# indianajohn/akaze-rust

Measured on AMD Instinct MI355X. Metric: Mpix/s through extract_features (4 oct x 4 sub), higher is better.
Workload: dtype f32

## Files before the change

### akaze-rust_amd/csrc/akz_kernels.hip

```cpp
#include <hip/hip_runtime.h>

#include <algorithm>
#include <cstdlib>

#include "akz_internal.hpp"
#include "akz_pm_g2.hpp"
#include "akz_libm.hpp"
#include "akz_prep_passes.hpp"

namespace akz {
namespace {

constexpr int BX = 64, BY = 4;

__device__ __forceinline__ int clampi(int v, int lo, int hi) { return v < lo ? lo : (v > hi ? hi : v); }

__device__ __forceinline__ float px(const float* p, long i) { return p[i]; }
__device__ __forceinline__ float px(const uint8_t* p, long i) { return ((float)p[i] * 1.0f) / 255.0f; }

template <typename T>
__global__ void k_filter_h(const T* __restrict__ in, float* __restrict__ out, int w, int h, Taps t) {
    const int x = blockIdx.x * BX + threadIdx.x, y = blockIdx.y * BY + threadIdx.y;
    if (x >= w || y >= h) return;
    const size_t base = (size_t)blockIdx.z * (size_t)w * (size_t)h;
// ... 319 lines not shown
            if (ly < n || ly >= n + TH || gy >= h || gx >= w) continue;
            const float* v = r == 0 ? la : lb;
            const float* st = r == 0 ? sta : stb;
            float* po = L_out + base + (size_t)gy * w;
            float* ps = Lstep ? Lstep + base + (size_t)gy * w : nullptr;
            if (vec_ok && gx + 3 < w) {
                plane_store4(po + gx, v[0], v[1], v[2], v[3]);
                if (ps) plane_store4(ps + gx, st[0], st[1], st[2], st[3]);
            } else {
#pragma unroll
                for (int e = 0; e < 4; ++e)
                    if (gx + e < w) {
                        plane_store(po + gx + e, v[e]);
                        if (ps) plane_store(ps + gx + e, st[e]);
                    }
            }
        }
    }
    if constexpr (EPI) {
        constexpr int IW = TW + 4, IH = TH + 4;
        static_assert(IH * IW + (TH + 4) * (TW + 2) + (TH + 2) * (TW + 2) <= 2 * PLANE, "the preparation's windows fit the two planes");
        float* const wI = sAB;
        float* const wA = wI + IH * IW;
        float* const wB = wA + (TH + 4) * (TW + 2);
        __syncthreads();
        if (active) {
#pragma unroll
            for (int r = 0; r < 2; ++r) {
                const int gy = r == 0 ? gya : gyb;
                const int wy = gy - (y0 - 2);
                if (wy < 0 || wy >= IH || gy < 0 || gy >= h) continue;
                const float* v = r == 0 ? la : lb;
#pragma unroll
                for (int e = 0; e < 4; ++e) {
                    const int wx = gx + e - (x0 - 2);
                    if (wx >= 0 && wx < IW && gx + e >= 0 && gx + e < w) wI[wy * IW + wx] = v[e];
                }
            }
        }
        __syncthreads();
        const double kc = octave_contrast(ep.d_k[blockIdx.z], ep.k_pow);
        prep_passes<TW, TH, NT>(wI, wA, wB, x0, y0, w, h, base, ep.lsmooth, ep.lflow, ep.taps, 1.0 / (kc * kc));
    }
}

__device__ __forceinline__ double grad_mod(const float* I, int w, int h, int x, int y, Scharr1 sk) {
    float lx, ly;
    scharr1_pair(I, w, h, x, y, sk, lx, ly);
    const double dx = (double)lx, dy = (double)ly;
    return sqrt(dx * dx + dy * dy);
}
constexpr int CT = 256;
__global__ void __launch_bounds__(CT)
k_contrast_max(const float* __restrict__ blurred, int w, int h, Scharr1 sk,
               unsigned long long* __restrict__ d_hmax_bits) {
    __shared__ unsigned long long s_part[CT / 64];
    const float* I = blurred + (size_t)blockIdx.z * (size_t)w * (size_t)h;
    double m = 0.0;
    for (int y = 1 + (int)blockIdx.x; y < h - 1; y += (int)gridDim.x)
        for (int x = 1 + (int)threadIdx.x; x < w - 1; x += CT) {
            const double g = grad_mod(I, w, h, x, y, sk);
            if (g > m) m = g;
        }
    unsigned long long bits = (unsigned long long)__double_as_longlong(m);
    for (int o = 32; o > 0; o >>= 1) {
        const unsigned long long other = __shfl_xor(bits, o, 64);
        bits = other > bits ? other : bits;
    }
    if ((threadIdx.x & 63) == 0) s_part[threadIdx.x >> 6] = bits;
    __syncthreads();
    if (threadIdx.x == 0) {
        for (int i = 1; i < CT / 64; ++i) bits = s_part[i] > bits ? s_part[i] : bits;
        if (bits != 0ull) atomicMax(d_hmax_bits + blockIdx.z, bits);
    }
}
__global__ void __launch_bounds__(CT)
k_contrast_hist(const float* __restrict__ blurred, int w, int h, Scharr1 sk,
                const unsigned long long* __restrict__ d_hmax_bits, unsigned nbins, unsigned copies,
                unsigned* __restrict__ d_hist) {
    extern __shared__ unsigned s_hist[];
    const unsigned tid = threadIdx.x;
    for (unsigned b = tid; b < nbins * copies; b += CT) s_hist[b] = 0u;
    __syncthreads();
    const float* I = blurred + (size_t)blockIdx.z * (size_t)w * (size_t)h;
    const double hmax = __longlong_as_double((long long)d_hmax_bits[blockIdx.z]);
    unsigned* mine = s_hist + (tid & (copies - 1u)) * nbins;
    for (int y = 1 + (int)blockIdx.x; y < h - 1; y += (int)gridDim.x)
        for (int x = 1 + (int)tid; x < w - 1; x += CT) {
            const double g = grad_mod(I, w, h, x, y, sk);
            if (g != 0.0) {
                const double f = floor((double)nbins * (g / hmax));
                const unsigned b = f >= (double)nbins ? nbins - 1u : (f > 0.0 ? (unsigned)f : 0u);
                atomicAdd(&mine[b], 1u);
            }
        }
    __syncthreads();
    for (unsigned b = tid; b < nbins; b += CT) {
        unsigned v = 0;
        for (unsigned c = 0; c < copies; ++c) v += s_hist[c * nbins + b];
        if (v) atomicAdd(&d_hist[(size_t)blockIdx.z * nbins + b], v);
    }
}
__device__ __forceinline__ unsigned long long sat_usize(double v) {
    if (!(v > 0.0)) return 0ull;
    if (v >= 18446744073709551615.0) return ~0ull;
    return (unsigned long long)v;
}
__global__ void __launch_bounds__(256)
k_contrast_final(const unsigned long long* __restrict__ d_hmax_bits, const unsigned* __restrict__ d_hist,
                 unsigned nbins, double percentile, unsigned n, double* __restrict__ d_k) {
    extern __shared__ unsigned s_bins[];
    const unsigned img = blockIdx.x;
    if (img >= n) return;
    const unsigned* hist = d_hist + (size_t)img * nbins;
    for (unsigned b = threadIdx.x; b < nbins; b += blockDim.x) s_bins[b] = hist[b];
    __syncthreads();
    if (threadIdx.x != 0) return;
    const double hmax = __longlong_as_double((long long)d_hmax_bits[img]);
    unsigned long long num_points = 0;
    for (unsigned b = 0; b < nbins; ++b) num_points += s_bins[b];
    const unsigned long long threshold = sat_usize((double)num_points * percentile);
    unsigned long long k = 0, num_elements = 0;
    while (num_elements < threshold && k < nbins) {
        num_elements += s_bins[k];
        k += 1;
    }
    d_k[img] = num_elements >= threshold ? hmax * (double)k / (double)nbins : 0.03;
}

template <int NTH>
__global__ void __launch_bounds__(NTH)
k_contrast_hist_final(const float* __restrict__ gxp, const float* __restrict__ gyp, int w, int h, unsigned long long* __restrict__ d_smax_bits,
                      unsigned nbins, unsigned copies, unsigned* __restrict__ d_hist, unsigned* __restrict__ d_done, double percentile,
                      double* __restrict__ d_k) {
    extern __shared__ unsigned s_hist[];
    __shared__ unsigned s_last;
    const unsigned tid = threadIdx.x, img = blockIdx.z;
    for (unsigned b = tid; b < nbins * copies; b += NTH) s_hist[b] = 0u;
    __syncthreads();
    const size_t px = (size_t)w * (size_t)h;
    const float* GX = gxp + (size_t)img * px;
    const float* GY = gyp + (size_t)img * px;
    const double hmax = sqrt(__longlong_as_double((long long)d_smax_bits[img]));
    unsigned* mine = s_hist + (tid & (copies - 1u)) * nbins;
    const bool vec = (px & 3u) == 0;
    const size_t nquads = (px + 3) / 4;
    for (size_t q = (size_t)blockIdx.x * NTH + tid; q < nquads; q += (size_t)gridDim.x * NTH) {
        const size_t i0 = q * 4;
        float ax[4], ay[4];
        if (vec) {
            const float4 a = *reinterpret_cast<const float4*>(GX + i0), b = *reinterpret_cast<const float4*>(GY + i0);
            ax[0] = a.x; ax[1] = a.y; ax[2] = a.z; ax[3] = a.w;
            ay[0] = b.x; ay[1] = b.y; ay[2] = b.z; ay[3] = b.w;
        } else {
#pragma unroll
            for (int e = 0; e < 4; ++e) {
                ax[e] = i0 + e < px ? GX[i0 + e] : 0.0f;
                ay[e] = i0 + e < px ? GY[i0 + e] : 0.0f;
            }
        }
        int y = (int)(i0 / (size_t)w), x = (int)(i0 - (size_t)y * w);
#pragma unroll
        for (int e = 0; e < 4; ++e) {
            if (x >= 1 && x < w - 1 && y >= 1 && y < h - 1) {
                const double dx = (double)ax[e], dy = (double)ay[e];
                const double g = sqrt(dx * dx + dy * dy);
                if (g != 0.0) {
                    const double f = floor((double)nbins * (g / hmax));
                    const unsigned b = f >= (double)nbins ? nbins - 1u : (f > 0.0 ? (unsigned)f : 0u);
                    atomicAdd(&mine[b], 1u);
                }
            }
            if (++x == w) {
                x = 0;
                ++y;
            }
        }
    }
    __syncthreads();
    unsigned* hist = d_hist + (size_t)img * nbins;
    for (unsigned b = tid; b < nbins; b += NTH) {
        unsigned v = 0;
        for (unsigned c = 0; c < copies; ++c) v += s_hist[c * nbins + b];
        if (v) {
            const unsigned before = atomicAdd(&hist[b], v);
            asm volatile("" ::"v"(before));
        }
    }
    __builtin_amdgcn_fence(__ATOMIC_RELEASE, "workgroup");
    __builtin_amdgcn_s_waitcnt(0);
    __syncthreads();
    if (tid == 0) s_last = atomicAdd(&d_done[img], 1u) == gridDim.x - 1u ? 1u : 0u;
    __syncthreads();
    if (!s_last) return;
    for (unsigned b = tid; b < nbins; b += NTH) {
        s_hist[b] = __hip_atomic_load(&hist[b], __ATOMIC_RELAXED, __HIP_MEMORY_SCOPE_AGENT);
        hist[b] = 0u;
    }
    __syncthreads();
    if (tid != 0) return;
    unsigned long long num_points = 0;
    for (unsigned b = 0; b < nbins; ++b) num_points += s_hist[b];
    const unsigned long long threshold = sat_usize((double)num_points * percentile);
    unsigned long long k = 0, num_elements = 0;
    while (num_elements < threshold && k < nbins) {
        num_elements += s_hist[k];
        k += 1;
    }
    d_k[img] = num_elements >= threshold ? hmax * (double)k / (double)nbins : 0.03;
    d_smax_bits[img] = 0ull;
    d_done[img] = 0u;
}
__global__ void __launch_bounds__(256)
k_flow_pair(const float* __restrict__ gxp, const float* __restrict__ gyp, float* __restrict__ lflow, size_t px, const double* __restrict__ d_k,
            unsigned k_pow) {
    const unsigned img = blockIdx.z;
    const double kc = octave_contrast(d_k[img], k_pow);
    const double inverse_k = 1.0 / (kc * kc);
    const float* GX = gxp + (size_t)img * px;
    const float* GY = gyp + (size_t)img * px;
    float* out = lflow + (size_t)img * px;
    const size_t i0 = ((size_t)blockIdx.x * 256 + threadIdx.x) * 4;
    if (i0 >= px) return;
    if ((px & 3u) == 0) {
        const float4 a = *reinterpret_cast<const float4*>(GX + i0), b = *reinterpret_cast<const float4*>(GY + i0);
        float4 o;
        o.x = pm_g2_px(a.x, b.x, inverse_k);
        o.y = pm_g2_px(a.y, b.y, inverse_k);
        o.z = pm_g2_px(a.z, b.z, inverse_k);
        o.w = pm_g2_px(a.w, b.w, inverse_k);
        *reinterpret_cast<float4*>(out + i0) = o;
    } else {
        for (size_t i = i0; i < i0 + 4 && i < px; ++i) out[i] = pm_g2_px(GX[i], GY[i], inverse_k);
    }
}

__global__ void k_ldet(const float* __restrict__ lxx, const float* __restrict__ lyy, const float* __restrict__ lxy,
                       float* __restrict__ out, size_t count, float q) {
    const size_t i = (size_t)blockIdx.x * blockDim.x + threadIdx.x;
    if (i >= count) return;
    out[i] = ((lxx[i] * lyy[i]) - (lxy[i] * lxy[i])) * q;
}

__global__ void k_accumulate(float* a, const float* b, size_t count) {
    const size_t i = (size_t)blockIdx.x * blockDim.x + threadIdx.x;
    if (i >= count) return;
    a[i] = a[i] + b[i];
}

__device__ __forceinline__ void nms_emit(float v, float xp, float xm, float yp, float ym, int x, int y, int w, int h,
                                         unsigned level, unsigned img, float thr, float border_m,
                                         Candidate* __restrict__ cand, unsigned cap, unsigned* __restrict__ count) {
    if (!(v > thr)) return;
    if (!(v > xp && v > xm && v > ym && v > yp)) return;
    const float fx = (float)x, fy = (float)y;
    const bool is_out = (roundf(fx - border_m) - 1.0f) < 0.0f || (roundf(fx + border_m) + 1.0f) >= (float)w ||
                        (roundf(fy - border_m) - 1.0f) < 0.0f || (roundf(fy + border_m) + 1.0f) >= (float)h;
    if (is_out) return;
    const unsigned slot = atomicAdd(count, 1u);
    if (slot < cap) {
        Candidate c;
        c.level = level;
        c.idx = (unsigned)(y * w + x);
        c.v = v; c.xp = xp; c.xm = xm; c.yp = yp; c.ym = ym;
        c.img = img;
        cand[slot] = c;
    }
}
__global__ void k_nms(const float* __restrict__ ldet, int w, int h, size_t img_stride, unsigned level, float thr,
                      float border_m, Candidate* __restrict__ cand, unsigned cap, unsigned* __restrict__ count) {
    const int x0 = (blockIdx.x * BX + threadIdx.x) * 4, y = blockIdx.y * BY + threadIdx.y;
    if (x0 >= w || y < 1 || y >= h - 1) return;
    const float* D = ldet + (size_t)blockIdx.z * img_stride;
    const float* row = D + (size_t)y * w;
    float c[6], up[4], dn[4];
    if ((w & 3) == 0 && x0 + 3 < w) {
        const float4 vc = *reinterpret_cast<const float4*>(row + x0);
        const float4 vu = *reinterpret_cast<const float4*>(row - w + x0);
        const float4 vd = *reinterpret_cast<const float4*>(row + w + x0);
        c[1] = vc.x; c[2] = vc.y; c[3] = vc.z; c[4] = vc.w;
        up[0] = vu.x; up[1] = vu.y; up[2] = vu.z; up[3] = vu.w;
        dn[0] = vd.x; dn[1] = vd.y; dn[2] = vd.z; dn[3] = vd.w;
    } else {
#pragma unroll
        for (int e = 0; e < 4; ++e) {
            const bool in = x0 + e < w;
            c[e + 1] = in ? row[x0 + e] : 0.0f;
            up[e] = in ? row[x0 + e - w] : 0.0f;
            dn[e] = in ? row[x0 + e + w] : 0.0f;
        }
    }
    c[0] = x0 > 0 ? row[x0 - 1] : 0.0f;
    c[5] = (x0 + 4 < w) ? row[x0 + 4] : 0.0f;
    const long last = (long)w * h - w - 1;
#pragma unroll
    for (int e = 0; e < 4; ++e) {
        const int x = x0 + e;
        if (x < 1 || x >= w) continue;
        if ((long)y * w + x >= last) continue;
        nms_emit(c[e + 1], c[e + 2], c[e], dn[e], up[e], x, y, w, h, level, blockIdx.z, thr, border_m, cand, cap, count);
    }
}

__constant__ float c_gauss25[7][7] = {
    {0.02546481f, 0.02350698f, 0.01849125f, 0.01239505f, 0.00708017f, 0.00344629f, 0.00142946f},
    {0.02350698f, 0.02169968f, 0.01706957f, 0.01144208f, 0.00653582f, 0.00318132f, 0.00131956f},
    {0.01849125f, 0.01706957f, 0.01342740f, 0.00900066f, 0.00514126f, 0.00250252f, 0.00103800f},
    {0.01239505f, 0.01144208f, 0.00900066f, 0.00603332f, 0.00344629f, 0.00167749f, 0.00069579f},
    {0.00708017f, 0.00653582f, 0.00514126f, 0.00344629f, 0.00196855f, 0.00095820f, 0.00039744f},
    {0.00344629f, 0.00318132f, 0.00250252f, 0.00167749f, 0.00095820f, 0.00046640f, 0.00019346f},
    {0.00142946f, 0.00131956f, 0.00103800f, 0.00069579f, 0.00039744f, 0.00019346f, 0.00008024f}};

struct OriTable {
    signed char a[112], b[112];
};
constexpr OriTable make_ori_table() {
    OriTable t{};
    int idx = 0;
    for (int i = -6; i <= 6; ++i)
        for (int j = -6; j <= 6; ++j)
            if (i * i + j * j < 36) {
                t.a[idx] = (signed char)i;
                t.b[idx] = (signed char)j;
                ++idx;
            }
    for (; idx < 112; ++idx) { t.a[idx] = 0; t.b[idx] = 0; }
    return t;
}
__constant__ OriTable c_ori = make_ori_table();
struct OriOrder {
    unsigned char k[112];
};
constexpr OriOrder make_ori_order() {
    OriOrder o{};
    const OriTable t = make_ori_table();
    int n = 0;
    for (int b = -6; b <= 6; ++b)
        for (int a = -6; a <= 6; ++a)
            for (int k = 0; k < 109; ++k)
                if (t.a[k] == a && t.b[k] == b) o.k[n++] = (unsigned char)k;
    for (; n < 112; ++n) o.k[n] = 0;
    return o;
}
__constant__ OriOrder c_ori_rows = make_ori_order();

__device__ __forceinline__ unsigned xcd_contiguous_group(unsigned b, unsigned nb) {
    return (b & 7u) * (nb >> 3) + (b >> 3);
}

constexpr int ORI_KPB = 32, ORI_NS = 109, ORI_NT = 256;
__global__ void __launch_bounds__(ORI_NT)
k_orientation(LevelTable tab, const KpParam* __restrict__ kps, unsigned nkp, const unsigned* __restrict__ d_nkp,
              unsigned long long window_mask, unsigned n_windows, OrientOut* __restrict__ out, unsigned out_stride) {
    __shared__ float s_rx[ORI_KPB * ORI_NS];
    __shared__ float s_ry[ORI_KPB * ORI_NS + 16];
    if (d_nkp) nkp = min(nkp, *d_nkp);
    const unsigned base = xcd_contiguous_group(blockIdx.x, gridDim.x) * ORI_KPB;
    if (base >= nkp) return;
    constexpr int ORI_IT = (ORI_KPB * ORI_NS + ORI_NT - 1) / ORI_NT, ORI_UB = 7;
    static_assert(ORI_IT % ORI_UB == 0, "whole batches");
    for (int it0 = 0; it0 < ORI_IT; it0 += ORI_UB) {
        float vx[ORI_UB], vy[ORI_UB], gw[ORI_UB];
        unsigned slot[ORI_UB];
#pragma unroll
        for (int u = 0; u < ORI_UB; ++u) {
            const unsigned idx = threadIdx.x + (unsigned)(it0 + u) * ORI_NT;
            const unsigned j = idx / ORI_NS, k = c_ori_rows.k[idx - j * ORI_NS];
            vx[u] = 0.0f; vy[u] = 0.0f; gw[u] = 0.0f;
            slot[u] = j * ORI_NS + k;
            if (idx < ORI_KPB * ORI_NS && base + j < nkp) {
                const KpParam kp = kps[base + j];
                const LevelPtrs lv = tab.lv[kp.level];
                const float* lx = lv.lx + (size_t)kp.img * lv.stride;
                const float* ly = lv.ly + (size_t)kp.img * lv.stride;
                const int a = c_ori.a[k], b = c_ori.b[k];
                const float fy = roundf(kp.yf + (float)b * kp.scale);
                const float fx = roundf(kp.xf + (float)a * kp.scale);
                const int iy = clampi(fy > 0.0f ? (int)fy : 0, 0, (int)lv.h - 1);
                const int ix = clampi(fx > 0.0f ? (int)fx : 0, 0, (int)lv.w - 1);
                gw[u] = c_gauss25[a < 0 ? -a : a][b < 0 ? -b : b];
                const size_t p = (size_t)iy * lv.w + ix;
                vx[u] = lx[p];
                vy[u] = ly[p];
            }
        }
#pragma unroll
        for (int u = 0; u < ORI_UB; ++u) {
            const unsigned idx = threadIdx.x + (unsigned)(it0 + u) * ORI_NT;
            const unsigned j = idx / ORI_NS;
            if (idx < ORI_KPB * ORI_NS) {
                const bool have = base + j < nkp;
                s_rx[slot[u]] = have ? gw[u] * vx[u] : 0.0f;
                s_ry[slot[u]] = have ? gw[u] * vy[u] : 0.0f;
            }
        }
    }
    __syncthreads();
    if (threadIdx.x >= 64) return;
    const unsigned lane = threadIdx.x, j = lane >> 1;
    const bool is_y = (lane & 1u) != 0;
    const float* py = s_ry + j * ORI_NS;
    const float* pa = is_y ? py : s_rx + j * ORI_NS;
    float t[ORI_NS];
#pragma unroll
    for (int k = 0; k < ORI_NS; ++k) t[k] = py[k] > 0.0f ? pa[k] : -0.0f;
    float sum = 0.0f, maxv = 0.0f, bx = 0.0f, by = 0.0f;
    unsigned found = 0;
    for (unsigned wdw = 0; wdw < n_windows; ++wdw) {
        if ((window_mask >> wdw) & 1ull) {
#pragma unroll
            for (int k = 0; k < ORI_NS; ++k) sum = sum + t[k];
        }
        const float other = __shfl_xor(sum, 1, 64);
        const float sx = is_y ? other : sum, sy = is_y ? sum : other;
        const float val = sx * sx + sy * sy;
        if (val > maxv) {
            maxv = val;
            bx = sx;
            by = sy;
            found = 1;
        }
    }
    if (!is_y && base + j < nkp) {
        OrientOut o;
        o.sum_x = bx; o.sum_y = by; o.found = found; o.angle_bits = 0;
        out[(size_t)(base + j) * out_stride] = o;
    }
}

struct PairTable {
    unsigned char a[162], b[162];
};
constexpr PairTable make_pairs() {
    PairTable t{};
    int p = 0;
    const int counts[3] = {4, 9, 16}, base[3] = {0, 4, 13};
    for (int g = 0; g < 3; ++g)
        for (int i = 0; i < counts[g]; ++i)
            for (int j = i + 1; j < counts[g]; ++j) {
                t.a[p] = (unsigned char)(base[g] + i);
                t.b[p] = (unsigned char)(base[g] + j);
                ++p;
            }
    return t;
}
__constant__ PairTable c_pairs = make_pairs();
struct BitTable3 {
    unsigned short e[512];
};
constexpr BitTable3 make_bits3() {
    BitTable3 t{};
    const PairTable p = make_pairs();
    const int npairs[3] = {6, 36, 120}, pbase[3] = {0, 6, 42};
    int b = 0;
    for (int g = 0; g < 3; ++g)
        for (int pos = 0; pos < 3; ++pos)
            for (int q = 0; q < npairs[g]; ++q)
                t.e[b++] = (unsigned short)((pos << 10) | (p.a[pbase[g] + q] << 5) | p.b[pbase[g] + q]);
    for (; b < 512; ++b) t.e[b] = 0;
    return t;
}
__constant__ BitTable3 c_bits3 = make_bits3();

constexpr int MLDB_KPB = 4;
constexpr int MLDB_LAT = 21, MLDB_NS = MLDB_LAT * MLDB_LAT;
struct DeviceAngles {
    OrientOut* sums;
    unsigned stride;
    unsigned fma;
    unsigned* flag;
};
struct MldbHostMirror {
    uint4* recs;
    const uint4* hdr;
    uint4* hdr_host;
    unsigned hdr_vec;
    uint8_t* desc;
};
__device__ __forceinline__ float2 device_angle(const DeviceAngles& da, unsigned kpi, bool write, const MldbHostMirror& hm) {
    OrientOut* o = da.sums + (size_t)kpi * da.stride;
    const float ang = o->found ? libm::atan2f_glibc(o->sum_y, o->sum_x) : 0.0f;
    bool bad = false;
    float co, si;
    if (da.fma) {
        co = libm::cosf_glibc<true>(ang, &bad);
        si = libm::sinf_glibc<true>(ang, &bad);
    } else {
        co = libm::cosf_glibc<false>(ang, &bad);
        si = libm::sinf_glibc<false>(ang, &bad);
    }
    if (write) {
        o->angle_bits = __float_as_uint(ang);
        if (bad && da.flag) atomicOr(da.flag, 1u);
        if (hm.recs) {
            const uint4* rec = reinterpret_cast<const uint4*>(da.sums) + (size_t)kpi * 2u - 1u;
            uint4 r0 = rec[0], r1 = rec[1];
            r1.w = __float_as_uint(ang);
            hm.recs[(size_t)kpi * 2u] = r0;
            hm.recs[(size_t)kpi * 2u + 1u] = r1;
        }
    }
    return float2{co, si};
}
__global__ void __launch_bounds__(64 * MLDB_KPB)
k_mldb(LevelTable tab, const KpParam* __restrict__ kps, const float2* __restrict__ cosi, unsigned nkp, const unsigned* __restrict__ d_nkp,
       DeviceAngles da, unsigned channels, uint8_t* __restrict__ desc64, unsigned first, MldbHostMirror hm) {
    __shared__ float s_win[MLDB_KPB][3][MLDB_NS + 7];
    __shared__ float s_val[MLDB_KPB][3][32];
    if (hm.recs && blockIdx.x == 0)
        for (unsigned i = threadIdx.x; i < hm.hdr_vec; i += 64 * MLDB_KPB) hm.hdr_host[i] = hm.hdr[i];
    if (d_nkp) nkp = min(nkp, *d_nkp);
    const unsigned lane = threadIdx.x & 63u, wv = threadIdx.x >> 6;
    const unsigned group0 = first + xcd_contiguous_group(blockIdx.x, gridDim.x) * MLDB_KPB;
    const unsigned kpi = group0 + wv;
    if (group0 >= nkp) return;
    const bool live = kpi < nkp;
    KpParam kp = kps[live ? kpi : 0];
    const float2 cs = da.sums ? device_angle(da, live ? kpi : 0, live && lane == 0, hm) : cosi[live ? kpi : 0];
    const LevelPtrs lv = tab.lv[__builtin_amdgcn_readfirstlane(kp.level)];
    const size_t ioff = (size_t)kp.img * lv.stride;
    const float* Lt = lv.lt + ioff;
    const float* Lx = lv.lx + ioff;
    const float* Ly = lv.ly + ioff;
    const float co = cs.x, si = cs.y, scale = kp.scale;
    unsigned short bits3[8];
#pragma unroll
    for (int r = 0; r < 8; ++r) bits3[r] = c_bits3.e[r * 64 + (int)lane];
    if (live) {
        constexpr int NIT = (MLDB_NS + 63) / 64;
        const bool k_fast = fabsf(co) >= fabsf(si);
        unsigned pidx[NIT];
        int widx[NIT];
#pragma unroll
        for (int it = 0; it < NIT; ++it) {
            const int sidx = min((int)lane + 64 * it, MLDB_NS - 1);
            const int qa = sidx / MLDB_LAT, qb = sidx - qa * MLDB_LAT;
            const int kk = k_fast ? qb : qa, ll = k_fast ? qa : qb;
            const int k = kk - 10, l = ll - 10;
            const float lf = (float)l + 0.5f, kf = (float)k + 0.5f;
            const float sample_y = kp.yf + (lf * co * scale + kf * si * scale);
            const float sample_x = kp.xf + (-lf * si * scale + kf * co * scale);
            const int y1 = clampi((int)roundf(sample_y), 0, (int)lv.h - 1);
            const int x1 = clampi((int)roundf(sample_x), 0, (int)lv.w - 1);
            pidx[it] = (unsigned)y1 * (unsigned)lv.w + (unsigned)x1;
            widx[it] = kk * MLDB_LAT + ll;
        }
        float vt[NIT], vx[NIT], vy[NIT];
#pragma unroll
        for (int it = 0; it < NIT; ++it) {
            vt[it] = Lt[pidx[it]];
            vx[it] = channels > 1 ? Lx[pidx[it]] : 0.0f;
            vy[it] = channels > 1 ? Ly[pidx[it]] : 0.0f;
        }
#pragma unroll
        for (int it = 0; it < NIT; ++it) {
            const int sidx = (int)lane + 64 * it;
            if (sidx >= MLDB_NS) continue;
            float v1 = 0.0f, v2 = 0.0f;
            if (channels > 1) {
                const float rx = vx[it], ry = vy[it];
                if (channels == 2) {
                    v1 = sqrtf(rx * rx + ry * ry);
                } else {
                    v2 = rx * co + ry * si;
                    v1 = -rx * si + ry * co;
                }
            }
            s_win[wv][0][widx[it]] = vt[it];
            s_win[wv][1][widx[it]] = v1;
            s_win[wv][2][widx[it]] = v2;
        }
    }
    __syncthreads();
    const unsigned cl = lane & 31u, ckp = 2u * wv + (lane >> 5);
    if (wv < MLDB_KPB / 2 && cl < 29 && group0 + ckp < nkp) {
        const int g = cl < 4 ? 0 : (cl < 13 ? 1 : 2);
        const int step = g == 0 ? 10 : (g == 1 ? 7 : 5), ng = g + 2;
        const int ci = (int)cl - (g == 0 ? 0 : (g == 1 ? 4 : 13));
        const int kk0 = (ci / ng) * step, ll0 = (ci % ng) * step;
        const int per_cell = step * step;
        const float* b0 = &s_win[ckp][0][0];
        const float* b1 = &s_win[ckp][1][0];
        const float* b2 = &s_win[ckp][2][0];
        float di = 0.0f, dx = 0.0f, dy = 0.0f;
#pragma unroll
        for (int dk = 0; dk < 10; ++dk) {
            const int o = (kk0 + min(dk, step - 1)) * MLDB_LAT + ll0;
            float r0[10], r1[10], r2[10];
#pragma unroll
            for (int dl = 0; dl < 10; ++dl) {
                r0[dl] = b0[o + dl];
                r1[dl] = b1[o + dl];
                r2[dl] = b2[o + dl];
            }
#pragma unroll
            for (int dl = 0; dl < 10; ++dl)
                if (dk < step && dl < step) {
                    di = di + r0[dl];
                    dx = dx + r1[dl];
                    dy = dy + r2[dl];
                }
        }
        const float ns = (float)per_cell;
        s_val[ckp][0][cl] = di / ns;
        s_val[ckp][1][cl] = dx / ns;
        s_val[ckp][2][cl] = dy / ns;
    }
    __syncthreads();
    const unsigned seg0 = 6u * channels, seg1 = seg0 + 36u * channels, total = seg1 + 120u * channels;
    unsigned long long words[8];
#pragma unroll
    for (int r = 0; r < 8; ++r) {
        const unsigned b = (unsigned)r * 64u + lane;
        bool bit = false;
        if (channels == 3) {
            const unsigned e = bits3[r];
            bit = s_val[wv][e >> 10][(e >> 5) & 31u] > s_val[wv][e >> 10][e & 31u];
        } else if (b < total) {
            unsigned rel, npairs, pbase;
            if (b < seg0) { rel = b; npairs = 6; pbase = 0; }
            else if (b < seg1) { rel = b - seg0; npairs = 36; pbase = 6; }
            else { rel = b - seg1; npairs = 120; pbase = 42; }
            const unsigned pos = rel / npairs, p = rel % npairs;
            bit = s_val[wv][pos][c_pairs.a[pbase + p]] > s_val[wv][pos][c_pairs.b[pbase + p]];
        }
        words[r] = __ballot(bit);
    }
    if (live && lane < 8) {
        unsigned long long wvw = words[0];
#pragma unroll
        for (int r = 1; r < 8; ++r)
            if (lane == (unsigned)r) wvw = words[r];
        reinterpret_cast<unsigned long long*>(desc64 + (size_t)kpi * 64)[lane] = wvw;
        if (hm.desc) reinterpret_cast<unsigned long long*>(hm.desc + (size_t)kpi * 64)[lane] = wvw;
    }
}

constexpr int MT = 256;

__device__ __forceinline__ unsigned hamming64(const uint4 (&q)[4], const uint4* __restrict__ row, unsigned tail_mask) {
    unsigned d = 0;
#pragma unroll
    for (int k = 0; k < 4; ++k) {
        const uint4 t = row[k];
        d += __popc(q[k].x ^ t.x);
        d += __popc(q[k].y ^ t.y);
        d += __popc(q[k].z ^ t.z);
        d += __popc((q[k].w ^ t.w) & (k == 3 ? tail_mask : 0xffffffffu));
    }
    return d;
}
__device__ __forceinline__ void top2_feed(unsigned d, unsigned j, unsigned& min_d, unsigned& second, unsigned& min_j) {
    if (d < min_d) {
        second = min_d;
        min_d = d;
        min_j = j;
    } else if (d < second) {
        second = d;
    }
}
__global__ void __launch_bounds__(MT) k_match(const uint4* __restrict__ d0, unsigned n0, const uint4* __restrict__ d1,
                                             unsigned n1, unsigned chunk_rows, unsigned threshold, unsigned tail_mask,
                                             MatchRec* __restrict__ out) {
    __shared__ uint4 s_tile[MT * 4];
    const unsigned i = blockIdx.x * MT + threadIdx.x;
    uint4 q[4];
    const bool live = i < n0;
#pragma unroll
    for (int k = 0; k < 4; ++k) q[k] = live ? d0[(size_t)i * 4 + k] : make_uint4(0, 0, 0, 0);
    unsigned min_d = threshold, second = threshold, min_j = 0;
    const unsigned begin = blockIdx.y * chunk_rows, end = min(n1, begin + chunk_rows);
    for (unsigned base = begin; base < end; base += MT) {
        const unsigned rows = min((unsigned)MT, end - base);
        __syncthreads();
        for (unsigned e = threadIdx.x; e < rows * 4; e += MT) s_tile[e] = d1[(size_t)base * 4 + e];
        __syncthreads();
        unsigned r = 0;
        for (; r + 4 <= rows; r += 4) {
            const unsigned da = hamming64(q, s_tile + (r + 0) * 4, tail_mask), db = hamming64(q, s_tile + (r + 1) * 4, tail_mask);
            const unsigned dc = hamming64(q, s_tile + (r + 2) * 4, tail_mask), dd = hamming64(q, s_tile + (r + 3) * 4, tail_mask);
            top2_feed(da, base + r + 0, min_d, second, min_j);
            top2_feed(db, base + r + 1, min_d, second, min_j);
            top2_feed(dc, base + r + 2, min_d, second, min_j);
            top2_feed(dd, base + r + 3, min_d, second, min_j);
        }
        for (; r < rows; ++r) top2_feed(hamming64(q, s_tile + r * 4, tail_mask), base + r, min_d, second, min_j);
    }
    if (live) {
        MatchRec m;
        m.min_d = min_d; m.second_d = second; m.min_j = min_j; m._pad = 0;
        out[(size_t)blockIdx.y * n0 + i] = m;
    }
}
__global__ void k_match_merge(const MatchRec* __restrict__ part, unsigned n0, unsigned chunks, unsigned threshold,
                              MatchRec* __restrict__ out) {
    const unsigned i = blockIdx.x * blockDim.x + threadIdx.x;
    if (i >= n0) return;
    unsigned min_d = threshold, second = threshold, min_j = 0;
    for (unsigned c = 0; c < chunks; ++c) {
        const MatchRec m = part[(size_t)c * n0 + i];
        top2_feed(m.min_d, m.min_j, min_d, second, min_j);
        if (m.second_d < second) second = m.second_d;
    }
    MatchRec o;
    o.min_d = min_d; o.second_d = second; o.min_j = min_j; o._pad = 0;
    out[i] = o;
}

__global__ void __launch_bounds__(1024) k_match_compact(const MatchRec* __restrict__ rec, unsigned n0, unsigned chunks,
                                                        unsigned threshold, double ratio2,
                                                        akz_match* __restrict__ out,
                                                        unsigned long long* __restrict__ n_out) {
    constexpr int IT = 16;
    __shared__ unsigned s_cnt[IT][16];
    __shared__ unsigned s_base;
    rec += (size_t)blockIdx.x * chunks * n0;
    out += (size_t)blockIdx.x * n0;
    n_out += blockIdx.x;
    const unsigned lane = threadIdx.x & 63u, wave = threadIdx.x >> 6;
    if (threadIdx.x == 0) s_base = 0;
    __syncthreads();
    for (unsigned start = 0; start < n0; start += IT * 1024u) {
        unsigned md[IT], mj[IT], keepmask = 0u;
#pragma unroll
        for (int it = 0; it < IT; ++it) {
            const unsigned i = start + (unsigned)it * 1024u + threadIdx.x;
            bool keep = false;
            md[it] = mj[it] = 0u;
            if (i < n0) {
                unsigned min_d = threshold, second = threshold, min_j = 0;
                for (unsigned c = 0; c < chunks; ++c) {
                    const MatchRec p = rec[(size_t)c * n0 + i];
                    top2_feed(p.min_d, p.min_j, min_d, second, min_j);
                    if (p.second_d < second) second = p.second_d;
                }
                md[it] = min_d; mj[it] = min_j;
                keep = ((double)min_d < (double)second * ratio2) && (min_d < threshold);
            }
            const unsigned long long bal = __ballot(keep);
            if (lane == 0) s_cnt[it][wave] = (unsigned)__popcll(bal);
            keepmask |= keep ? 1u << it : 0u;
        }
        __syncthreads();
        unsigned off = s_base;
#pragma unroll
        for (int it = 0; it < IT; ++it) {
            unsigned row = 0, below = 0;
#pragma unroll
            for (unsigned w = 0; w < 16; ++w) {
                const unsigned c = s_cnt[it][w];
                row += c;
                below += w < wave ? c : 0u;
            }
            const bool keep = (keepmask >> it) & 1u;
            const unsigned long long bal = __ballot(keep);
            if (keep) {
                akz_match o;
                o.index_0 = start + (unsigned)it * 1024u + threadIdx.x; o.index_1 = mj[it]; o.distance = (double)md[it];
                out[off + below + (unsigned)__popcll(bal & ((1ull << lane) - 1ull))] = o;
            }
            off += row;
        }
        __syncthreads();
        if (threadIdx.x == 0) s_base = off;
        __syncthreads();
    }
    if (threadIdx.x == 0) *n_out = s_base;
}

__global__ void __launch_bounds__(256) k_match_merge_compact(const MatchRec* __restrict__ part, unsigned n0, unsigned chunks,
                                                             unsigned threshold, double ratio2, akz_match* __restrict__ out,
                                                             unsigned long long* __restrict__ n_out,
                                                             unsigned long long* __restrict__ state, unsigned epoch) {
    __shared__ unsigned s_cnt[4];
    __shared__ unsigned s_prefix;
    const unsigned b = blockIdx.x, tid = threadIdx.x, lane = tid & 63u, wave = tid >> 6;
    const unsigned i = b * 256u + tid;
    unsigned min_d = threshold, second = threshold, min_j = 0;
    bool keep = false;
    if (i < n0) {
        for (unsigned c = 0; c < chunks; ++c) {
            const MatchRec m = part[(size_t)c * n0 + i];
            top2_feed(m.min_d, m.min_j, min_d, second, min_j);
            if (m.second_d < second) second = m.second_d;
        }
        keep = ((double)min_d < (double)second * ratio2) && (min_d < threshold);
    }
    const unsigned long long bal = __ballot(keep);
    if (lane == 0) s_cnt[wave] = (unsigned)__popcll(bal);
    __syncthreads();
    const unsigned total = s_cnt[0] + s_cnt[1] + s_cnt[2] + s_cnt[3];
    unsigned below = 0;
    for (unsigned w = 0; w < wave; ++w) below += s_cnt[w];
    if (tid == 0)
        __hip_atomic_store(state + b, ((unsigned long long)epoch << 32) | total, __ATOMIC_RELAXED, __HIP_MEMORY_SCOPE_AGENT);
    if (wave == 0) {
        unsigned sum = 0;
        for (unsigned j0 = 0; j0 < b; j0 += 64u) {
            const unsigned j = j0 + lane;
            unsigned v = 0;
            if (j < b) {
                unsigned long long w;
                do {
                    w = __hip_atomic_load(state + j, __ATOMIC_RELAXED, __HIP_MEMORY_SCOPE_AGENT);
                } while ((unsigned)(w >> 32) != epoch);
                v = (unsigned)w;
            }
            for (int o = 32; o > 0; o >>= 1) v += __shfl_xor(v, o, 64);
            sum += v;
        }
        if (lane == 0) s_prefix = sum;
    }
    __syncthreads();
    const unsigned prefix = s_prefix;
    if (keep) {
        akz_match o;
        o.index_0 = i; o.index_1 = min_j; o.distance = (double)min_d;
        out[prefix + below + (unsigned)__popcll(bal & ((1ull << lane) - 1ull))] = o;
    }
    if (b == gridDim.x - 1 && tid == 0) *n_out = (unsigned long long)prefix + total;
}

inline dim3 grid2d(uint32_t w, uint32_t h, uint32_t n) { return dim3((w + BX - 1) / BX, (h + BY - 1) / BY, n); }

}

namespace launch {

static Scharr1 scharr1() {
    const Taps m = taps_scharr_main(1);
    return Scharr1{m.wgt[0], m.wgt[1]};
}

void filter_h_f32(hipStream_t s, const float* in, float* out, uint32_t w, uint32_t h, uint32_t n, const Taps& t) {
    hipLaunchKernelGGL(k_filter_h<float>, grid2d(w, h, n), dim3(BX, BY), 0, s, in, out, (int)w, (int)h, t);
}
void filter_h_u8(hipStream_t s, const uint8_t* in, float* out, uint32_t w, uint32_t h, uint32_t n, const Taps& t) {
    hipLaunchKernelGGL(k_filter_h<uint8_t>, grid2d(w, h, n), dim3(BX, BY), 0, s, in, out, (int)w, (int)h, t);
}
void filter_v_f32(hipStream_t s, const float* in, float* out, uint32_t w, uint32_t h, uint32_t n, const Taps& t) {
    hipLaunchKernelGGL(k_filter_v, grid2d(w, h, n), dim3(BX, BY), 0, s, in, out, (int)w, (int)h, t);
}
void delay(hipStream_t s, uint32_t microseconds) {
    hipLaunchKernelGGL(k_delay, dim3(1), dim3(64), 0, s, (unsigned long long)microseconds * 100ull, (unsigned*)nullptr);
}
void half_size(hipStream_t s, const float* in, float* out, uint32_t w, uint32_t h, uint32_t n) {
    if ((w & 7u) == 0 && (((uintptr_t)in | (uintptr_t)out) & 15u) == 0) {
        hipLaunchKernelGGL(k_half_size4, grid2d(w / 4, h / 2, n), dim3(BX, BY), 0, s, in, out, (int)w, (int)h);
        return;
    }
    hipLaunchKernelGGL(k_half_size, grid2d(w / 2, h / 2, n), dim3(BX, BY), 0, s, in, out, (int)w, (int)h);
}
void pm_g2(hipStream_t s, const float* lx, const float* ly, float* out, uint32_t w, uint32_t h, uint32_t n,
           const double* d_k, uint32_t k_scale_pow) {
    const size_t plane = (size_t)w * h;
    hipLaunchKernelGGL(k_pm_g2, dim3((unsigned)((plane + 255) / 256), 1, n), dim3(256), 0, s, lx, ly, out, plane, d_k,
                       k_scale_pow);
}
void flow(hipStream_t s, const float* lsmooth, float* lflow, uint32_t w, uint32_t h, uint32_t n, const double* d_k,
          uint32_t k_scale_pow) {
    hipLaunchKernelGGL(k_flow, grid2d(w, h, n), dim3(BX, BY), 0, s, lsmooth, lflow, (int)w, (int)h, scharr1(), d_k,
                       k_scale_pow);
}
void fed_step(hipStream_t s, const float* lt_in, const float* lflow, float* lt_out, float* lstep, uint32_t w,
              uint32_t h, uint32_t n, float half_tau) {
    hipLaunchKernelGGL(k_fed_step, grid2d(w, h, n), dim3(BX, BY), 0, s, lt_in, lflow, lt_out, lstep, (int)w, (int)h,
                       half_tau);
}
constexpr int kFedDeepTh = 10;
uint64_t fed_deep_workgroups(uint32_t w, uint32_t h, uint32_t n) {
    return (uint64_t)((w + 63) / 64) * ((h + kFedDeepTh - 1) / kFedDeepTh) * n;
}
bool fed_epilogue_supported(uint32_t w, uint32_t h, uint32_t n_steps) {
    if (n_steps == 0 || n_steps > 14 || w < 8 || h < 8 || (w - 1) % 64 == 0) return false;
    const uint32_t th = n_steps <= 6 ? 32u : (uint32_t)kFedDeepTh;
    return (h - 1) % th != 0;
}
void fed_fused(hipStream_t s, const float* lt_in, const float* lflow, float* lt_out, float* lstep, uint32_t w,
               uint32_t h, uint32_t n, const float* half_taus, uint32_t n_steps, const FedNextPrep* next) {
    constexpr int TW = 64, TH = 32, NT = 512;
    FedTaus ht;
    ht.n = (int)n_steps;
    for (uint32_t i = 0; i < 16; ++i) ht.half_tau[i] = i < n_steps ? half_taus[i] : 0.0f;
    const dim3 grid((w + TW - 1) / TW, (h + TH - 1) / TH, n);
    FedEpi ep{};
    if (next) {
        const Taps m = taps_scharr_main(1);
        ep.lsmooth = next->lsmooth;
        ep.lflow = next->lflow;
        ep.taps = PrepTaps{next->g3[0], next->g3[1], next->g3[2], m.wgt[0], m.wgt[1]};
        ep.d_k = next->d_k;
        ep.k_pow = next->k_pow;
        if (n_steps <= 6) {
            hipLaunchKernelGGL((k_fed_own<TW, TH, 8, NT, true>), grid, dim3(NT), 0, s, lt_in, lflow, lt_out, lstep, (int)w, (int)h, ht, ep);
        } else {
            const dim3 g10((w + TW - 1) / TW, (h + kFedDeepTh - 1) / kFedDeepTh, n);
            hipLaunchKernelGGL((k_fed_own<TW, kFedDeepTh, 16, NT, true>), g10, dim3(NT), 0, s, lt_in, lflow, lt_out, lstep, (int)w, (int)h, ht,
                               ep);
        }
        return;
    }
    {
        if (n_steps <= 4) {
            if (h >= 48) {
                const dim3 g48((w + TW - 1) / TW, (h + 47) / 48, n);
                hipLaunchKernelGGL((k_fed_own<TW, 48, 4, NT>), g48, dim3(NT), 0, s, lt_in, lflow, lt_out, lstep, (int)w,
                                   (int)h, ht, ep);
            } else
                hipLaunchKernelGGL((k_fed_own<TW, TH, 4, NT>), grid, dim3(NT), 0, s, lt_in, lflow, lt_out, lstep, (int)w,
// ... 137 lines not shown
```

Measured before the change: 15060.

## Stage orientation keypoint params in LDS and specialize MLDB cell means per grid

The orientation kernel now loads each keypoint's level pointers and parameters once into shared memory, and packs sample offsets with their Gaussian weights into one constant table copied to LDS. This removes the per-sample global KpParam and LevelTable loads and the nkp predicate; out-of-range keypoints clamp to the last valid one. It also adds a scheduling barrier so all gathers are issued before use. In MLDB, cell averaging is split so each wave handles one grid size for all keypoints through templated fixed-step loops, replacing a padded 10x10 loop with step masks, at the cost of more branch code.

```diff
diff --git a/akaze-rust_amd/csrc/akz_kernels.hip b/akaze-rust_amd/csrc/akz_kernels.hip
--- a/akaze-rust_amd/csrc/akz_kernels.hip
+++ b/akaze-rust_amd/csrc/akz_kernels.hip
@@ -645,7 +645,7 @@
     }
 }
 
-__constant__ float c_gauss25[7][7] = {
+constexpr float k_gauss25[7][7] = {
     {0.02546481f, 0.02350698f, 0.01849125f, 0.01239505f, 0.00708017f, 0.00344629f, 0.00142946f},
     {0.02350698f, 0.02169968f, 0.01706957f, 0.01144208f, 0.00653582f, 0.00318132f, 0.00131956f},
     {0.01849125f, 0.01706957f, 0.01342740f, 0.00900066f, 0.00514126f, 0.00250252f, 0.00103800f},
@@ -670,36 +670,72 @@
     for (; idx < 112; ++idx) { t.a[idx] = 0; t.b[idx] = 0; }
     return t;
 }
-__constant__ OriTable c_ori = make_ori_table();
-struct OriOrder {
-    unsigned char k[112];
+struct alignas(8) OriSample {
+    float gw;
+    signed char a, b;
+    unsigned char k, _pad;
 };
-constexpr OriOrder make_ori_order() {
-    OriOrder o{};
+struct OriSamples {
+    OriSample s[112];
+};
+constexpr OriSamples make_ori_samples() {
+    OriSamples o{};
     const OriTable t = make_ori_table();
     int n = 0;
     for (int b = -6; b <= 6; ++b)
         for (int a = -6; a <= 6; ++a)
             for (int k = 0; k < 109; ++k)
-                if (t.a[k] == a && t.b[k] == b) o.k[n++] = (unsigned char)k;
-    for (; n < 112; ++n) o.k[n] = 0;
+                if (t.a[k] == a && t.b[k] == b) {
+                    o.s[n].gw = k_gauss25[a < 0 ? -a : a][b < 0 ? -b : b];
+                    o.s[n].a = (signed char)a;
+                    o.s[n].b = (signed char)b;
+                    o.s[n].k = (unsigned char)k;
+                    o.s[n]._pad = 0;
+                    ++n;
+                }
+    for (; n < 112; ++n) o.s[n] = OriSample{0.0f, 0, 0, 0, 0};
     return o;
 }
-__constant__ OriOrder c_ori_rows = make_ori_order();
+__constant__ OriSamples c_ori_samples = make_ori_samples();
 
 __device__ __forceinline__ unsigned xcd_contiguous_group(unsigned b, unsigned nb) {
     return (b & 7u) * (nb >> 3) + (b >> 3);
 }
 
 constexpr int ORI_KPB = 32, ORI_NS = 109, ORI_NT = 256;
+struct alignas(8) OriKp {
+    const float* lx;
+    const float* ly;
+    int w, h;
+    float xf, yf, scale;
+    unsigned _pad;
+};
+using GlobalFloats = const __attribute__((address_space(1))) float*;
 __global__ void __launch_bounds__(ORI_NT)
 k_orientation(LevelTable tab, const KpParam* __restrict__ kps, unsigned nkp, const unsigned* __restrict__ d_nkp,
               unsigned long long window_mask, unsigned n_windows, OrientOut* __restrict__ out, unsigned out_stride) {
     __shared__ float s_rx[ORI_KPB * ORI_NS];
     __shared__ float s_ry[ORI_KPB * ORI_NS + 16];
+    __shared__ OriKp s_kp[ORI_KPB];
+    __shared__ OriSample s_sm[112];
     if (d_nkp) nkp = min(nkp, *d_nkp);
     const unsigned base = xcd_contiguous_group(blockIdx.x, gridDim.x) * ORI_KPB;
     if (base >= nkp) return;
+    if (threadIdx.x < ORI_KPB) {
+        const KpParam kp = kps[min(base + threadIdx.x, nkp - 1u)];
+        const LevelPtrs lv = tab.lv[kp.level];
+        OriKp k;
+        k.lx = lv.lx + (size_t)kp.img * lv.stride;
+        k.ly = lv.ly + (size_t)kp.img * lv.stride;
+        k.w = (int)lv.w;
+        k.h = (int)lv.h;
+        k.xf = kp.xf; k.yf = kp.yf; k.scale = kp.scale;
+        k._pad = 0u;
+        s_kp[threadIdx.x] = k;
+    } else if (threadIdx.x >= 64 && threadIdx.x < 64 + 112) {
+        s_sm[threadIdx.x - 64] = c_ori_samples.s[threadIdx.x - 64];
+    }
+    __syncthreads();
     constexpr int ORI_IT = (ORI_KPB * ORI_NS + ORI_NT - 1) / ORI_NT, ORI_UB = 7;
     static_assert(ORI_IT % ORI_UB == 0, "whole batches");
     for (int it0 = 0; it0 < ORI_IT; it0 += ORI_UB) {
@@ -707,34 +743,30 @@
         unsigned slot[ORI_UB];
 #pragma unroll
         for (int u = 0; u < ORI_UB; ++u) {
-            const unsigned idx = threadIdx.x + (unsigned)(it0 + u) * ORI_NT;
-            const unsigned j = idx / ORI_NS, k = c_ori_rows.k[idx - j * ORI_NS];
-            vx[u] = 0.0f; vy[u] = 0.0f; gw[u] = 0.0f;
-            slot[u] = j * ORI_NS + k;
-            if (idx < ORI_KPB * ORI_NS && base + j < nkp) {
-                const KpParam kp = kps[base + j];
-                const LevelPtrs lv = tab.lv[kp.level];
-                const float* lx = lv.lx + (size_t)kp.img * lv.stride;
-                const float* ly = lv.ly + (size_t)kp.img * lv.stride;
-                const int a = c_ori.a[k], b = c_ori.b[k];
-                const float fy = roundf(kp.yf + (float)b * kp.scale);
-                const float fx = roundf(kp.xf + (float)a * kp.scale);
-                const int iy = clampi(fy > 0.0f ? (int)fy : 0, 0, (int)lv.h - 1);
-                const int ix = clampi(fx > 0.0f ? (int)fx : 0, 0, (int)lv.w - 1);
-                gw[u] = c_gauss25[a < 0 ? -a : a][b < 0 ? -b : b];
-                const size_t p = (size_t)iy * lv.w + ix;
-                vx[u] = lx[p];
-                vy[u] = ly[p];
-            }
-        }
+            const unsigned idx = min(threadIdx.x + (unsigned)(it0 + u) * ORI_NT, (unsigned)(ORI_KPB * ORI_NS - 1));
+            const unsigned j = idx / ORI_NS;
+            const OriSample sm = s_sm[idx - j * ORI_NS];
+            const OriKp kp = s_kp[j];
+            gw[u] = sm.gw;
+            slot[u] = j * ORI_NS + sm.k;
+            const int a = sm.a, b = sm.b;
+            const float fy = roundf(kp.yf + (float)b * kp.scale);
+            const float fx = roundf(kp.xf + (float)a * kp.scale);
+            const int iy = clampi(fy > 0.0f ? (int)fy : 0, 0, kp.h - 1);
+            const int ix = clampi(fx > 0.0f ? (int)fx : 0, 0, kp.w - 1);
+            const size_t p = (size_t)iy * (unsigned)kp.w + ix;
+            vx[u] = ((GlobalFloats)kp.lx)[p];
+            vy[u] = ((GlobalFloats)kp.ly)[p];
+        }
+        __builtin_amdgcn_sched_barrier(0);
+#pragma unroll
+        for (int u = 0; u < ORI_UB; ++u) asm volatile("" : "+v"(vx[u]), "+v"(vy[u]));
 #pragma unroll
         for (int u = 0; u < ORI_UB; ++u) {
             const unsigned idx = threadIdx.x + (unsigned)(it0 + u) * ORI_NT;
-            const unsigned j = idx / ORI_NS;
             if (idx < ORI_KPB * ORI_NS) {
-                const bool have = base + j < nkp;
-                s_rx[slot[u]] = have ? gw[u] * vx[u] : 0.0f;
-                s_ry[slot[u]] = have ? gw[u] * vy[u] : 0.0f;
+                s_rx[slot[u]] = gw[u] * vx[u];
+                s_ry[slot[u]] = gw[u] * vy[u];
             }
         }
     }
@@ -746,7 +778,10 @@
     const float* pa = is_y ? py : s_rx + j * ORI_NS;
     float t[ORI_NS];
 #pragma unroll
-    for (int k = 0; k < ORI_NS; ++k) t[k] = py[k] > 0.0f ? pa[k] : -0.0f;
+    for (int k = 0; k < ORI_NS; ++k) {
+        const float y = py[k], a = pa[k];
+        t[k] = y > 0.0f ? a : -0.0f;
+    }
     float sum = 0.0f, maxv = 0.0f, bx = 0.0f, by = 0.0f;
     unsigned found = 0;
     for (unsigned wdw = 0; wdw < n_windows; ++wdw) {
@@ -807,6 +842,8 @@
 
 constexpr int MLDB_KPB = 4;
 constexpr int MLDB_LAT = 21, MLDB_NS = MLDB_LAT * MLDB_LAT;
+constexpr int MLDB_WIN = MLDB_NS + 7;
+static_assert(16 * MLDB_KPB <= 64 && MLDB_KPB >= 3, "k_mldb: a grid's cells of all keypoints are lanes of one wave, one wave per grid");
 struct DeviceAngles {
     OrientOut* sums;
     unsigned stride;
@@ -845,10 +882,34 @@
     }
     return float2{co, si};
 }
+template <int STEP>
+__device__ __forceinline__ void mldb_cell_means(const float* __restrict__ win, int o, float* __restrict__ val) {
+    float di = 0.0f, dx = 0.0f, dy = 0.0f;
+#pragma unroll
+    for (int dk = 0; dk < STEP; ++dk) {
+        float r0[STEP], r1[STEP], r2[STEP];
+#pragma unroll
+        for (int dl = 0; dl < STEP; ++dl) {
+            r0[dl] = win[o + dk * MLDB_LAT + dl];
+            r1[dl] = win[MLDB_WIN + o + dk * MLDB_LAT + dl];
+            r2[dl] = win[2 * MLDB_WIN + o + dk * MLDB_LAT + dl];
+        }
+#pragma unroll
+        for (int dl = 0; dl < STEP; ++dl) {
+            di = di + r0[dl];
+            dx = dx + r1[dl];
+            dy = dy + r2[dl];
+        }
+    }
+    constexpr float ns = (float)(STEP * STEP);
+    val[0] = di / ns;
+    val[32] = dx / ns;
+    val[64] = dy / ns;
+}
 __global__ void __launch_bounds__(64 * MLDB_KPB)
 k_mldb(LevelTable tab, const KpParam* __restrict__ kps, const float2* __restrict__ cosi, unsigned nkp, const unsigned* __restrict__ d_nkp,
        DeviceAngles da, unsigned channels, uint8_t* __restrict__ desc64, unsigned first, MldbHostMirror hm) {
-    __shared__ float s_win[MLDB_KPB][3][MLDB_NS + 7];
+    __shared__ float s_win[MLDB_KPB][3 * MLDB_WIN];
     __shared__ float s_val[MLDB_KPB][3][32];
     if (hm.recs && blockIdx.x == 0)
         for (unsigned i = threadIdx.x; i < hm.hdr_vec; i += 64 * MLDB_KPB) hm.hdr_host[i] = hm.hdr[i];
@@ -909,45 +970,27 @@
                     v1 = -rx * si + ry * co;
                 }
             }
-            s_win[wv][0][widx[it]] = vt[it];
-            s_win[wv][1][widx[it]] = v1;
-            s_win[wv][2][widx[it]] = v2;
-        }
-    }
-    __syncthreads();
-    const unsigned cl = lane & 31u, ckp = 2u * wv + (lane >> 5);
-    if (wv < MLDB_KPB / 2 && cl < 29 && group0 + ckp < nkp) {
-        const int g = cl < 4 ? 0 : (cl < 13 ? 1 : 2);
-        const int step = g == 0 ? 10 : (g == 1 ? 7 : 5), ng = g + 2;
-        const int ci = (int)cl - (g == 0 ? 0 : (g == 1 ? 4 : 13));
-        const int kk0 = (ci / ng) * step, ll0 = (ci % ng) * step;
-        const int per_cell = step * step;
-        const float* b0 = &s_win[ckp][0][0];
-        const float* b1 = &s_win[ckp][1][0];
-        const float* b2 = &s_win[ckp][2][0];
-        float di = 0.0f, dx = 0.0f, dy = 0.0f;
-#pragma unroll
-        for (int dk = 0; dk < 10; ++dk) {
-            const int o = (kk0 + min(dk, step - 1)) * MLDB_LAT + ll0;
-            float r0[10], r1[10], r2[10];
-#pragma unroll
-            for (int dl = 0; dl < 10; ++dl) {
-                r0[dl] = b0[o + dl];
-                r1[dl] = b1[o + dl];
-                r2[dl] = b2[o + dl];
-            }
-#pragma unroll
-            for (int dl = 0; dl < 10; ++dl)
-                if (dk < step && dl < step) {
-                    di = di + r0[dl];
-                    dx = dx + r1[dl];
-                    dy = dy + r2[dl];
-                }
-        }
-        const float ns = (float)per_cell;
-        s_val[ckp][0][cl] = di / ns;
-        s_val[ckp][1][cl] = dx / ns;
-        s_val[ckp][2][cl] = dy / ns;
+            s_win[wv][widx[it]] = vt[it];
+            s_win[wv][MLDB_WIN + widx[it]] = v1;
+            s_win[wv][2 * MLDB_WIN + widx[it]] = v2;
+        }
+    }
+    __syncthreads();
+    {
+        const unsigned grid = __builtin_amdgcn_readfirstlane(wv) & 3u;
+        const int ng = (int)grid + 2, cells = ng * ng;
+        const int ckp = ((int)lane >= cells) + ((int)lane >= 2 * cells) + ((int)lane >= 3 * cells) + ((int)lane >= 4 * cells);
+        const int ci = (int)lane - ckp * cells;
+        if (grid < 3u && ckp < MLDB_KPB && group0 + (unsigned)ckp < nkp) {
+            const float* win = &s_win[ckp][0];
+            const int ck = ci / ng, cc = ci - ck * ng;
+            if (grid == 0u)
+                mldb_cell_means<10>(win, ck * 10 * MLDB_LAT + cc * 10, &s_val[ckp][0][ci]);
+            else if (grid == 1u)
+                mldb_cell_means<7>(win, ck * 7 * MLDB_LAT + cc * 7, &s_val[ckp][0][4 + ci]);
+            else
+                mldb_cell_means<5>(win, ck * 5 * MLDB_LAT + cc * 5, &s_val[ckp][0][13 + ci]);
+        }
     }
     __syncthreads();
     const unsigned seg0 = 6u * channels, seg1 = seg0 + 36u * channels, total = seg1 + 120u * channels;
```

Result: no change. 15100, median of 6 (+0.3%).
